# sen-ye/dmvae

Measured on AMD Instinct MI355X. Metric: images/sec DMVAE train step @256x256, higher is better.
Workload: dtype bf16

## Files before the change

dmvae_amd/csrc/conv_pp.hip:

```cpp
#include "common.h"
#include "dmvae_hip.h"
#include <cstdlib>
#include <atomic>
#include <mutex>
#include <type_traits>
#include <unordered_map>


namespace dmvae_conv_pp {

struct Args {
  const bf16* x;
  const bf16* w;
  const float* bias;
  const bf16* res;
  void* y;
  int N, Hi, Wi, Cin, Ho, Wo, Cout;
  int ks, act, M, ctiles, total;
  int so, pd, sd;
  int Ml;
  unsigned wsRow, wsTap, wsChunk;
  float* gnpart;
  unsigned* sched;
  unsigned long long* dbg;
};

__device__ __forceinline__ int hswz(int row) { return (row >> 1) & 2; }

__device__ __forceinline__ void divmod_small(int m, int d, float inv_d, bool, int& q, int& r) {
  q = (int)((float)m * inv_d);
  r = m - q * d;
  if (r < 0) { q--; r += d; }
  if (r >= d) { q++; r -= d; }
}

template <int TM, int TP, int WM, int WP, int NBUF, bool UPS, bool OUT_F32, bool KO, bool GEN = false, bool SUB = false, bool DYN = false, bool STATS = false,
          bool HALO = false>
__global__ __launch_bounds__(512) void conv_pp_kernel(Args a) {
#if __HIP_DEVICE_COMPILE__
  constexpr int BM = TM / WM / 32, BP = TP / WP / 32;
  constexpr int TILE_A = TM * 64, TILE_B = TP * 64, SLOT = TILE_A + TILE_B;
  constexpr int NPA = TM >= 128 ? TM / 128 : 1, NPB = TP / 128;
  static_assert(TM >= 128 || HALO, "the 64-row tile exists in the halo form only");
  constexpr int NP = NPA + NPB;
  constexpr int PF = NBUF - 1;
  static_assert(WM * WP == 8 && BM * BP == 8, "8 waves x 8 accumulators");
  static_assert(!HALO || (!UPS && !GEN && !SUB && KO && NBUF == 4), "HALO: plain 3x3, chunk-outer K order");
  constexpr int NPH = NPB + 1;
  constexpr int HALO_B = (TP + 16) * 64;
  constexpr int GROUP = 2 * TILE_A + HALO_B;
  constexpr int EPI_OFF = HALO ? GROUP : 2 * SLOT;
  constexpr int EPI_BYTES = 8 * 32 * (((BM >= 4 ? BM / 2 : BM) * 32) * 4 + 16);
  constexpr int DUMP_OFF = GROUP + (GROUP > EPI_BYTES ? GROUP : EPI_BYTES);
  constexpr bool DIRECT = HALO && !OUT_F32;
  constexpr int BM16 = BM * 2, BP16 = BP * 2;
  extern __shared__ __attribute__((aligned(16))) char smem[];

  const int tid = threadIdx.x, lane = tid & 63;
  const int wave = __builtin_amdgcn_readfirstlane(tid >> 6);
  const int grp = wave >> 2;
  const int wm = wave / WP, wp = wave % WP;
  static_assert(!SUB || (!UPS && !GEN && KO), "SUB: its own instantiation, chunk-outer K order");
  const int T = SUB ? 4 : a.ks * a.ks;
  const int TW = SUB ? 16 : T;
  const int nchunk = a.Cin >> 5;
  const int nK = T * nchunk;

  const unsigned wbytes = (unsigned)a.Cout * TW * a.Cin * 2u;
  const unsigned xbytes = (unsigned)a.N * a.Hi * a.Wi * a.Cin * 2u;
  const int SR = GEN ? ((UPS || a.ks == 1) ? 0 : (a.sd == 2 ? 1 : a.pd)) : 1;
  const int sds = GEN && a.sd == 2 ? 1 : 0;
  const unsigned shift = GEN ? ((!UPS && a.ks != 1) ? (unsigned)(SR * a.Wi + SR) * a.Cin * 2u : 0u)
                             : ((!UPS && (SUB || a.ks == 3)) ? (unsigned)(a.Wi + 1) * a.Cin * 2u : 0u);
  const __amdgpu_buffer_rsrc_t rA = dmvae_buffer_rsrc(a.w, wbytes);
  const __amdgpu_buffer_rsrc_t rB =
      dmvae_buffer_rsrc(reinterpret_cast<const char*>(a.x) - shift, xbytes + shift);

  const int dvw = SUB ? a.Wi : a.Wo;
  const int hw = SUB ? a.Hi * a.Wi : a.Ho * a.Wo;
  const float inv_hw = 1.0f / (float)hw, inv_wo = 1.0f / (float)dvw;
  const bool small_m = a.M < (1 << 24);
  int m0 = 0, n0 = 0;
  int par = 0;
  unsigned voffA[NPA];
  unsigned ctrB[NPB], maskB[NPB], selB[NPB];
  unsigned rowo[UPS ? NPB : 1][3], colo[UPS ? NPB : 1][3];
  unsigned ctrH[HALO ? NPH : 1], mskH[HALO ? NPH : 1];
  int it_ky = 0;
  int it = 0, it_tap = 0, it_ch = 0;
  unsigned soffB_tap = 0;
  auto setup = [&](unsigned work) {
    int lane_s = lane;
    if constexpr (DIRECT) asm volatile("" : "+v"(lane_s));
    const unsigned wid = xcd_remap(work, a.total);
    if constexpr (SUB) {
      const unsigned q = wid / a.ctiles;
      n0 = (int)(wid - q * a.ctiles) * TM;
      par = __builtin_amdgcn_readfirstlane((int)(q & 3u));
      m0 = (int)(q >> 2) * TP;
    } else {
      m0 = (int)(wid / a.ctiles) * TP;
      n0 = (int)(wid % a.ctiles) * TM;
    }
    it = it_tap = it_ch = 0;
    it_ky = 0;
#pragma unroll
    for (int p = 0; p < NPA; p++) {
      const int row = (wave * NPA + p) * 16 + (lane_s >> 2);
      int co = n0 + row;
      if constexpr (DIRECT) {
        constexpr int CW_ = TM / WM;
        const int wmr = row / CW_, rr = row % CW_;
        co = n0 + wmr * CW_ + BM16 * (rr & 15) + (rr >> 4);
      }
      const int c = (lane_s & 3) ^ swz64(row);
      voffA[p] = (co < a.Cout && row < TM) ? (unsigned)co * a.wsRow + c * 16u : SENT;
    }
    if constexpr (HALO) {
#pragma unroll
      for (int q = 0; q < NPH; q++) {
        const int i = (q < NPB ? (wave * NPB + q) * 16 : TP) + (lane_s >> 2);
        const int own = min(max(i - 1, 0), TP - 1);
        const int m = m0 + own;
        const int c = (lane_s & 3) ^ hswz(i);
        unsigned mask = 0;
        if (m < a.M && i < TP + 2 && (q < NPB || wave == 0)) {
          int n, r, y, x;
          divmod_small(m, hw, inv_hw, small_m, n, r);
          divmod_small(r, dvw, inv_wo, small_m, y, x);
          mask = (y > 0 ? 1u : 0u) | 2u | (y < a.Ho - 1 ? 4u : 0u);
          if ((i == 0 && x == 0) || (i == TP + 1 && x == a.Wo - 1)) mask = 0;
        }
        ctrH[q] = (unsigned)(m0 + i) * a.Cin * 2u + c * 16u;
        mskH[q] = mask;
      }
    } else {
#pragma unroll
    for (int p = 0; p < NPB; p++) {
    const int row = (wave * NPB + p) * 16 + (lane_s >> 2);
    const int m = m0 + row;
    const int c = (lane_s & 3) ^ swz64(row);
    unsigned mask = 0;
    ctrB[p] = 0;
    if (m < a.M) {
      int n, r, y, x;
      divmod_small(m, hw, inv_hw, small_m, n, r);
      divmod_small(r, dvw, inv_wo, small_m, y, x);
      int by = y, bx = x;
      if constexpr (SUB) {
        by = y - 1 + (par >> 1); bx = x - 1 + (par & 1);
        const unsigned rm = (by >= 0 ? 0x3u : 0u) | (by + 1 < a.Hi ? 0xCu : 0u);
        const unsigned cm = (bx >= 0 ? 0x5u : 0u) | (bx + 1 < a.Wi ? 0xAu : 0u);
        mask = rm & cm;
      } else if (UPS || !GEN) {
        if (a.ks == 3) {
          const unsigned rm = (y > 0 ? 0x007u : 0u) | 0x038u | (y < a.Ho - 1 ? 0x1C0u : 0u);
          const unsigned cm = (x > 0 ? 0x049u : 0u) | 0x092u | (x < a.Wo - 1 ? 0x124u : 0u);
          mask = rm & cm;
        } else {
          mask = 1;
        }
      } else if (a.ks == 1) {
        mask = 1;
      } else {
        const int y0 = y * a.so - a.pd, x0 = x * a.so - a.pd;
        by = sds ? (y0 + 1) >> 1 : y0;
        bx = sds ? (x0 + 1) >> 1 : x0;
        unsigned rmk = 0, cmk = 0;
#pragma unroll
        for (int k = 0; k < 4; k++) {
          if (k < a.ks) {
            const bool ry = sds ? (((y0 + k) & 1) == 0 && (unsigned)(by + (k >> 1)) < (unsigned)a.Hi) : (unsigned)(by + k) < (unsigned)a.Hi;
            const bool rx = sds ? (((x0 + k) & 1) == 0 && (unsigned)(bx + (k >> 1)) < (unsigned)a.Wi) : (unsigned)(bx + k) < (unsigned)a.Wi;
            rmk |= (unsigned)ry << k;
            cmk |= (unsigned)rx << k;
          }
        }
#pragma unroll
        for (int k = 0; k < 4; k++)
          if (k < a.ks && ((rmk >> k) & 1u)) mask |= cmk << (k * a.ks);
      }
      if (UPS) {
#pragma unroll
        for (int k = 0; k < 3; k++) {
          const int yy = min(max(y + k - 1, 0), a.Ho - 1) >> 1, xx = min(max(x + k - 1, 0), a.Wo - 1) >> 1;
          rowo[UPS ? p : 0][k] = (unsigned)((n * a.Hi + yy) * a.Wi) * a.Cin * 2u + c * 16u;
          colo[UPS ? p : 0][k] = (unsigned)xx * a.Cin * 2u;
        }
        if (a.ks != 3) ctrB[p] = rowo[UPS ? p : 0][1] + colo[UPS ? p : 0][1];
      } else {
        if constexpr (GEN) ctrB[p] = (unsigned)((n * a.Hi + by + SR) * a.Wi + bx + SR) * a.Cin * 2u + c * 16u;
        else if constexpr (SUB) ctrB[p] = (unsigned)((n * a.Hi + by + 1) * a.Wi + bx + 1) * a.Cin * 2u + c * 16u;
        else ctrB[p] = (unsigned)((n * a.Hi + y) * a.Wi + x) * a.Cin * 2u + c * 16u;
      }
    }
    maskB[p] = mask;
    selB[p] = SENT;
  }
    }
  };

  const int kg = lane >> 5;
  int aoff[BM16], boff[BP16];
#pragma unroll
  for (int i = 0; i < BM16; i++) {
    const int row = wm * (TM / WM) + i * 16 + (lane & 15);
    aoff[i] = row * 64 + (((lane >> 4) ^ swz64(row)) << 4);
  }
#pragma unroll
  for (int j = 0; j < BP16; j++) {
    const int row = wp * (TP / WP) + j * 16 + (lane & 15);
    boff[j] = TILE_A + row * 64 + (((lane >> 4) ^ swz64(row)) << 4);
  }

  f32x4 acc[BM16][BP16];

  auto new_tap = [&]() {
    int ky, kx;
    if constexpr (GEN) {
      ky = a.ks == 3 ? it_tap / 3 : (a.ks == 4 ? it_tap >> 2 : 1); kx = a.ks == 3 ? it_tap - (it_tap / 3) * 3 : (a.ks == 4 ? it_tap & 3 : 1);
      soffB_tap = (!UPS && a.ks != 1) ? (unsigned)((ky >> sds) * a.Wi + (kx >> sds)) * a.Cin * 2u : 0u;
    } else if constexpr (SUB) {
      ky = it_tap >> 1; kx = it_tap & 1;
      soffB_tap = (unsigned)(ky * a.Wi + kx) * a.Cin * 2u;
    } else {
      ky = a.ks == 3 ? it_tap / 3 : 1; kx = a.ks == 3 ? it_tap - (it_tap / 3) * 3 : 1;
      soffB_tap = (!UPS && a.ks == 3) ? (unsigned)(ky * a.Wi + kx) * a.Cin * 2u : 0u;
    }
#pragma unroll
    for (int p = 0; p < NPB; p++) {
      unsigned v = ctrB[p];
      if (UPS && a.ks == 3) {
        const unsigned ro = ky == 0 ? rowo[UPS ? p : 0][0] : (ky == 1 ? rowo[UPS ? p : 0][1] : rowo[UPS ? p : 0][2]);
        const unsigned co = kx == 0 ? colo[UPS ? p : 0][0] : (kx == 1 ? colo[UPS ? p : 0][1] : colo[UPS ? p : 0][2]);
        v = ro + co;
      }
      selB[p] = ((maskB[p] >> it_tap) & 1u) ? v : SENT;
    }
  };
  auto issue = [&](int slot) {
    const bool live = it < nK;
    if (live && (KO || it_ch == 0)) new_tap();
    unsigned soA = (unsigned)it_tap * a.wsTap + (unsigned)it_ch * a.wsChunk;
    if constexpr (SUB)
      soA = (unsigned)((((par >> 1) + (it_tap & 2)) << 2) + (par & 1) + ((it_tap & 1) << 1)) * a.wsTap + (unsigned)it_ch * a.wsChunk;
    unsigned soB = soffB_tap + (unsigned)it_ch * 64u;
    constexpr bool live_b = true;
    if constexpr (GEN) {
      soA = (unsigned)__builtin_amdgcn_readfirstlane((int)soA);
      soB = (unsigned)__builtin_amdgcn_readfirstlane((int)soB);
    }
#pragma unroll
    for (int p = 0; p < NPA; p++)
      __builtin_amdgcn_raw_ptr_buffer_load_lds(rA, LPTR(smem + slot + (wave * NPA + p) * 1024), 16, live ? voffA[p] : SENT, soA, 0, 0);
#pragma unroll
    for (int p = 0; p < NPB; p++)
      __builtin_amdgcn_raw_ptr_buffer_load_lds(rB, LPTR(smem + slot + TILE_A + (wave * NPB + p) * 1024), 16, (live && live_b) ? selB[p] : SENT, soB, 0, 0);
    it++;
    if (KO) {
      if (++it_tap == T) { it_tap = 0; it_ch++; }
    } else {
      if (++it_ch == nchunk) { it_ch = 0; it_tap++; }
    }
  };

  auto issue_h = [&](auto KXc) __attribute__((always_inline)) {
    constexpr int KX = decltype(KXc)::value;
    const bool live = it < nK;
    const unsigned soA = (unsigned)(it_ky * 3 + KX) * a.wsTap + (unsigned)it_ch * a.wsChunk;
    const int isl = it;
    const int da = ((isl >> 1) & 1) * GROUP + (isl & 1) * TILE_A;
#pragma unroll
    for (int p = 0; p < NPA; p++)
      __builtin_amdgcn_raw_ptr_buffer_load_lds(rA, LPTR(smem + ((wave * NPA + p) * 16 < TM ? da + (wave * NPA + p) * 1024 : DUMP_OFF)), 16, live ? voffA[p] : SENT, soA, 0, 0);
    if constexpr (KX == 0) {
      const unsigned soH = (unsigned)(it_ky * a.Wi) * a.Cin * 2u + (unsigned)it_ch * 64u;
      const int dh = ((it_ch + it_ky) & 1) * GROUP + 2 * TILE_A;
#pragma unroll
      for (int q = 0; q < NPH; q++) {
        const unsigned v = (live && ((mskH[HALO ? q : 0] >> it_ky) & 1u)) ? ctrH[HALO ? q : 0] : SENT;
        const int dst = q < NPB ? dh + (wave * NPB + q) * 1024 : (wave == 0 ? dh + TP * 64 : DUMP_OFF);
        __builtin_amdgcn_raw_ptr_buffer_load_lds(rB, LPTR(smem + dst), 16, v, soH, 0, 0);
      }
    }
    it++;
    if constexpr (KX == 2) {
      if (++it_ky == 3) { it_ky = 0; it_ch++; }
    }
  };
  using K0_ = std::integral_constant<int, 0>; using K1_ = std::integral_constant<int, 1>; using K2_ = std::integral_constant<int, 2>;

  auto stamp = [&](unsigned work, int k) {
    if (a.dbg && tid == 0) a.dbg[(size_t)work * 8 + k] = __builtin_amdgcn_s_memtime();
  };
  auto claim = [&]() {
    if (tid == 0) {
      const unsigned x = blockIdx.x & 7u, first = gridDim.x >> 3;
      unsigned flat = 0xFFFFFFFFu;
      for (unsigned k = 0; k < 8u; k++) {
        const unsigned xx = (x + k) & 7u;
        const unsigned cnt = ((unsigned)a.total >> 3) + (xx < ((unsigned)a.total & 7u) ? 1u : 0u);
        const unsigned j = first + atomicAdd(a.sched + xx, 1u);
        if (j < cnt) { flat = j * 8u + xx; break; }
      }
      __hip_atomic_store(a.sched + 16 + blockIdx.x, flat, __ATOMIC_RELEASE, __HIP_MEMORY_SCOPE_WORKGROUP);
    }
  };
  stamp(blockIdx.x, 0);
  setup(blockIdx.x);
  stamp(blockIdx.x, 1);
  if constexpr (HALO) {
    issue_h(K0_{}); issue_h(K1_{}); issue_h(K2_{});
  } else {
#pragma unroll
    for (int u = 0; u < PF; u++) issue(u * SLOT);
  }
  for (unsigned work = blockIdx.x; work < (unsigned)a.total;) {
  const int m0c = m0, n0c = n0;
  const int parc = par;
  if constexpr (DYN) claim();
  int boffk[HALO ? 3 : 1][HALO ? BP16 : 1];
  if constexpr (HALO) {
    int lane_h = lane;
    asm volatile("" : "+v"(lane_h));
#pragma unroll
    for (int j = 0; j < BP16; j++) {
      const int prow = wp * (TP / WP) + j * 16 + (lane_h & 15);
      int q, x;
      divmod_small(m0c + prow, dvw, inv_wo, small_m, q, x);
      const int zoff = (TP + 2) * 64 + ((lane_h >> 4) << 4);
#pragma unroll
      for (int k = 0; k < 3; k++) {
        const int h = prow + k;
        const int off = h * 64 + (((lane_h >> 4) ^ hswz(h)) << 4);
        boffk[HALO ? k : 0][HALO ? j : 0] = (k == 0 && x == 0) || (k == 2 && x == a.Wo - 1) ? zoff : off;
      }
    }
  }
#pragma unroll
  for (int i = 0; i < BM16; i++)
#pragma unroll
    for (int j = 0; j < BP16; j++)
#pragma unroll
      for (int r = 0; r < 4; r++) acc[i][j][r] = 0.f;
  wait_vmcnt<HALO ? 2 * NPA : (PF - 1) * NP>();
  __builtin_amdgcn_s_barrier();
  stamp(work, 2);
  if (grp == 1) __builtin_amdgcn_s_setprio(1);
  if (grp == 1) __builtin_amdgcn_s_barrier();

  bf16x8 af[BM16], bfr[BP16];
  int slot_rd = 0, slot_wr = PF * SLOT;
  unsigned next_dyn = 0;
  if constexpr (HALO) {
    int ka = 0, sh = 2 * TILE_A;
    auto ktile = [&](auto KXc) __attribute__((always_inline)) {
      constexpr int KX = decltype(KXc)::value;
      const char* sa = smem + ((ka >> 1) & 1) * GROUP + (ka & 1) * TILE_A;
      const char* sb = smem + sh;
#pragma unroll
      for (int j = 0; j < BP16; j++) bfr[j] = *reinterpret_cast<const bf16x8*>(sb + boffk[HALO ? KX : 0][HALO ? j : 0]);
#pragma unroll
      for (int i = 0; i < BM16; i++) af[i] = *reinterpret_cast<const bf16x8*>(sa + aoff[i]);
      issue_h(KXc);
      ka++;
      if constexpr (KX == 2) sh = sh == 2 * TILE_A ? GROUP + 2 * TILE_A : 2 * TILE_A;
      wait_vmcnt<KX == 2 ? 2 * NPA : 2 * NPA + NPH>();
      __builtin_amdgcn_s_waitcnt(0xC07F);
      asm volatile("" ::: "memory");
      __builtin_amdgcn_sched_barrier(0);
      __builtin_amdgcn_s_barrier();
      __builtin_amdgcn_sched_barrier(0);
#pragma unroll
      for (int i = 0; i < BM16; i++)
#pragma unroll
        for (int j = 0; j < BP16; j++) {
          if constexpr (DIRECT) asm volatile("v_mfma_f32_16x16x32_bf16 %0, %1, %2, %0" : "+a"(acc[i][j]) : "v"(bfr[j]), "v"(af[i]));
          else asm volatile("v_mfma_f32_16x16x32_bf16 %0, %1, %2, %0" : "+a"(acc[i][j]) : "v"(af[i]), "v"(bfr[j]));
        }
      __builtin_amdgcn_sched_barrier(0);
      __builtin_amdgcn_s_barrier();
      __builtin_amdgcn_sched_barrier(0);
    };
#pragma unroll 1
    for (int t = 0; t < nK; t += 3) { ktile(K0_{}); ktile(K1_{}); ktile(K2_{}); }
  } else {
#pragma unroll 1
  for (int t = 0; t < nK; t++) {
    const char* sb = smem + slot_rd;
#pragma unroll
    for (int j = 0; j < BP16; j++) bfr[j] = *reinterpret_cast<const bf16x8*>(sb + boff[j]);
#pragma unroll
    for (int i = 0; i < BM16; i++) af[i] = *reinterpret_cast<const bf16x8*>(sb + aoff[i]);
    issue(slot_wr);
    slot_rd = slot_rd + SLOT == NBUF * SLOT ? 0 : slot_rd + SLOT;
    slot_wr = slot_wr + SLOT == NBUF * SLOT ? 0 : slot_wr + SLOT;
    wait_vmcnt<(PF - 1) * NP>();
    __builtin_amdgcn_s_waitcnt(0xC07F);
    asm volatile("" ::: "memory");
    __builtin_amdgcn_sched_barrier(0);
    __builtin_amdgcn_s_barrier();
    __builtin_amdgcn_sched_barrier(0);
#pragma unroll
    for (int i = 0; i < BM16; i++)
#pragma unroll
      for (int j = 0; j < BP16; j++)
        asm volatile("v_mfma_f32_16x16x32_bf16 %0, %1, %2, %0" : "+a"(acc[i][j]) : "v"(af[i]), "v"(bfr[j]));
    __builtin_amdgcn_sched_barrier(0);
    __builtin_amdgcn_s_barrier();
    __builtin_amdgcn_sched_barrier(0);
  }
  }
  stamp(work, 3);
  if (grp == 0) __builtin_amdgcn_s_barrier();
  if constexpr (DYN) next_dyn = __hip_atomic_load(a.sched + 16 + blockIdx.x, __ATOMIC_ACQUIRE, __HIP_MEMORY_SCOPE_WORKGROUP);
  wait_vmcnt<0>();
  asm volatile("s_nop 15\n\ts_nop 15" ::: "memory");

  __builtin_amdgcn_s_barrier();
  stamp(work, 6);
  const unsigned next = DYN ? (unsigned)__builtin_amdgcn_readfirstlane((int)next_dyn) : work + gridDim.x;
  const bool has_next = next < (unsigned)a.total;
  if constexpr (DIRECT) {
    typedef unsigned u32x4 __attribute__((ext_vector_type(4)));
    typedef unsigned u32x2 __attribute__((ext_vector_type(2)));
    constexpr int CL = BM16;
    constexpr int NQD = CL / 4;
    static_assert(CL == 8 || CL == 4, "DIRECT: 8 or 4 couts per lane");
    int lane_o = lane;
    asm volatile("" : "+v"(lane_o));
    const int cc = lane_o & 15, gq = lane_o >> 4;
    const int col = n0c + wm * (TM / WM) + CL * cc;
    const bool c_ok = col < a.Cout;
    const __amdgpu_buffer_rsrc_t rY = dmvae_buffer_rsrc(a.y, (unsigned)a.M * (unsigned)a.Cout * 2u);
    const __amdgpu_buffer_rsrc_t rBias = dmvae_buffer_rsrc(a.bias, a.bias ? (unsigned)a.Cout * 4u : 0u);
    float bsv[CL];
    {
      const unsigned vo = c_ok ? (unsigned)col * 4u : SENT;
#pragma unroll
      for (int h = 0; h < NQD; h++) {
        const u32x4 b4 = __builtin_amdgcn_raw_buffer_load_b128(rBias, vo == SENT ? SENT : vo + 16u * h, 0, 0);
        const f32x4 bf = *reinterpret_cast<const f32x4*>(&b4);
#pragma unroll
        for (int e = 0; e < 4; e++) bsv[4 * h + e] = bf[e];
      }
    }
    if (has_next) {
      stamp(next, 0);
      setup(next);
      stamp(next, 1);
    } else {
      it = (nK + 3) & ~3;
      it_ky = it_ch = 0;
    }
    issue_h(K0_{});
    stamp(work, 7);
    float s1[STATS ? NQD : 1], s2[STATS ? NQD : 1];
    if constexpr (STATS) {
#pragma unroll
      for (int h = 0; h < NQD; h++) { s1[h] = 0.f; s2[h] = 0.f; }
    }
    const unsigned vbase = c_ok ? ((unsigned)(m0c + wp * (TP / WP) + 4 * gq) * (unsigned)a.Cout + (unsigned)col) * 2u : SENT;
    const unsigned rstep = (unsigned)a.Cout * 2u;
    auto body = [&](auto RESc, auto ACTc) __attribute__((always_inline)) {
      constexpr bool RES = decltype(RESc)::value;
      constexpr int ACTC = decltype(ACTc)::value;
      const __amdgpu_buffer_rsrc_t rR = dmvae_buffer_rsrc(a.res, RES ? (unsigned)a.M * (unsigned)a.Cout * 2u : 0u);
      typedef std::conditional_t<CL == 8, u32x4, u32x2> rvec;
      rvec rnx[RES ? 4 : 1];
      auto fetch = [&](int j, int r) {
        if constexpr (RES) {
          if constexpr (CL == 8) rnx[RES ? r : 0] = __builtin_amdgcn_raw_buffer_load_b128(rR, vbase, (unsigned)(j * 16 + r) * rstep, 2);
          else rnx[RES ? r : 0] = __builtin_amdgcn_raw_buffer_load_b64(rR, vbase, (unsigned)(j * 16 + r) * rstep, 2);
        }
      };
#pragma unroll
      for (int r = 0; r < 4; r++) fetch(0, r);
#pragma unroll
      for (int j = 0; j < BP16; j++) {
#pragma unroll
        for (int r = 0; r < 4; r++) {
          float v[CL];
#pragma unroll
          for (int i = 0; i < CL; i++) {
            float x;
            asm volatile("v_accvgpr_read_b32 %0, %1" : "=v"(x) : "a"(acc[i][j][r]));
            v[i] = x + bsv[i];
          }
          const int act = ACTC >= 0 ? ACTC : a.act;
          if constexpr (RES) {
            float rf[CL];
            {
              const rvec rv = rnx[RES ? r : 0];
#pragma unroll
              for (int h = 0; h < CL / 2; h++) {
                const unsigned wd = rv[h];
                const bf16x2 b2 = *reinterpret_cast<const bf16x2*>(&wd);
                rf[2 * h] = (float)b2[0]; rf[2 * h + 1] = (float)b2[1];
              }
            }
            if (j + 1 < BP16) fetch(j + 1, r);
            if (act == 3) {
#pragma unroll
              for (int e = 0; e < CL; e++) v[e] = rf[e] > 0.f ? v[e] : 0.f;
            } else {
#pragma unroll
              for (int e = 0; e < CL; e++) v[e] += rf[e];
            }
          }
          if (act == 1) {
#pragma unroll
            for (int e = 0; e < CL; e++) v[e] = v[e] * sigmoidf_(v[e]);
          } else if (act == 2) {
#pragma unroll
            for (int e = 0; e < CL; e++) v[e] = v[e] > 0.f ? v[e] : 0.f;
          } else if (act == 4) {
#pragma unroll
            for (int e = 0; e < CL; e++) v[e] = v[e] > 0.f ? v[e] : 0.2f * v[e];
          }
          const unsigned so = (unsigned)(j * 16 + r) * rstep;
          unsigned pk[CL / 2];
#pragma unroll
          for (int h = 0; h < CL / 2; h++) pk[h] = dmvae_pack_bf16x2(v[2 * h], v[2 * h + 1]);
          if constexpr (STATS) {
            const bf16x2 one2 = {(bf16)1.0f, (bf16)1.0f};
#pragma unroll
            for (int h = 0; h < CL / 2; h++) {
              const bf16x2 p2 = *reinterpret_cast<const bf16x2*>(&pk[h]);
              s1[STATS ? h >> 1 : 0] = __builtin_amdgcn_fdot2_f32_bf16(p2, one2, s1[STATS ? h >> 1 : 0], false);
              s2[STATS ? h >> 1 : 0] = __builtin_amdgcn_fdot2_f32_bf16(p2, p2, s2[STATS ? h >> 1 : 0], false);
            }
          }
          if constexpr (CL == 8) {
            const u32x4 o = {pk[0], pk[1], pk[2], pk[3]};
            __builtin_amdgcn_raw_buffer_store_b128(o, rY, vbase, so, 2 );
            asm volatile("s_nop 0" :: "v"(o));
          } else {
            const u32x2 o = {pk[0], pk[1]};
            __builtin_amdgcn_raw_buffer_store_b64(o, rY, vbase, so, 2 );
            asm volatile("s_nop 0" :: "v"(o));
          }
        }
      }
    };
    using T_ = std::true_type; using F_ = std::false_type;
    if (a.res) {
      if (a.act == 0) body(T_{}, std::integral_constant<int, 0>{});
      else if (a.act == 3) body(T_{}, std::integral_constant<int, 3>{});
      else body(T_{}, std::integral_constant<int, -1>{});
    } else {
      if (a.act == 0) body(F_{}, std::integral_constant<int, 0>{});
      else if (a.act == 2) body(F_{}, std::integral_constant<int, 2>{});
      else body(F_{}, std::integral_constant<int, -1>{});
    }
    if constexpr (STATS) {
      const size_t trow = (size_t)(m0c / TP) * WP + wp;
#pragma unroll
      for (int h = 0; h < NQD; h++) {
        float t1 = s1[STATS ? h : 0], t2 = s2[STATS ? h : 0];
        t1 += __shfl_xor(t1, 16, 64); t2 += __shfl_xor(t2, 16, 64);
        t1 += __shfl_xor(t1, 32, 64); t2 += __shfl_xor(t2, 32, 64);
        const int cq = col + 4 * h;
        if (gq == 0 && cq < a.Cout) *reinterpret_cast<f32x2*>(a.gnpart + (trow * (a.Cout >> 2) + (cq >> 2)) * 2) = f32x2{t1, t2};
      }
    }
  } else {
    constexpr int EH = BM >= 4 ? BM / 2 : BM;
    constexpr int NH = BM / EH;
    constexpr int CWH = EH * 32;
    constexpr int ROWB = CWH * 4 + 16;
    constexpr int LPR = CWH / 8, RPI = 64 / LPR;
    constexpr int NI = 32 / RPI;
    constexpr unsigned ES = OUT_F32 ? 4u : 2u;
    static_assert(!STATS || !OUT_F32, "STATS: statistics of the bf16 result");
    typedef unsigned u32x4 __attribute__((ext_vector_type(4)));
    char* reg = smem + EPI_OFF + wave * (32 * ROWB);
    int lane_o = lane;
    asm volatile("" : "+v"(lane_o));
    const int cl = lane_o % LPR, rg = lane_o / LPR;
    const unsigned mout = SUB ? 4u * (unsigned)a.M : (unsigned)a.M;
    const __amdgpu_buffer_rsrc_t rY = dmvae_buffer_rsrc(a.y, mout * (unsigned)a.Cout * ES);
    const __amdgpu_buffer_rsrc_t rBias = dmvae_buffer_rsrc(a.bias, a.bias ? (unsigned)a.Cout * 4u : 0u);
    f32x4 bias_lo[NH], bias_hi[NH];
#pragma unroll
    for (int hh = 0; hh < NH; hh++) {
      const int cb = n0c + wm * (TM / WM) + hh * CWH + cl * 8;
      const unsigned vo = cb < a.Cout ? (unsigned)cb * 4u : SENT;
      const u32x4 b0 = __builtin_amdgcn_raw_buffer_load_b128(rBias, vo, 0, 0), b1 = __builtin_amdgcn_raw_buffer_load_b128(rBias, vo + 16u, 0, 0);
      bias_lo[hh] = *reinterpret_cast<const f32x4*>(&b0);
      bias_hi[hh] = *reinterpret_cast<const f32x4*>(&b1);
    }
    if (has_next) {
      stamp(next, 0);
      setup(next);
      stamp(next, 1);
    } else {
      it = HALO ? (nK + 3) & ~3 : nK;
      it_ky = it_ch = 0;
    }
    if constexpr (HALO) issue_h(K0_{}); else issue(0);
    stamp(work, 7);
    float sacc[STATS ? NH : 1][2][2];
    if constexpr (STATS) {
#pragma unroll
      for (int i = 0; i < NH * 4; i++) (&sacc[0][0][0])[i] = 0.f;
    }
    auto body = [&](auto RESc, auto ACTc) __attribute__((always_inline)) {
      constexpr bool RES = decltype(RESc)::value;
      constexpr int ACTC = decltype(ACTc)::value;
      const __amdgpu_buffer_rsrc_t rR = dmvae_buffer_rsrc(a.res, RES ? mout * (unsigned)a.Cout * 2u : 0u);
#pragma unroll
      for (int hh = 0; hh < NH; hh++) {
        if (n0c + wm * (TM / WM) + hh * CWH >= a.Cout) continue;
        const int cb = n0c + wm * (TM / WM) + hh * CWH + cl * 8;
        const bool c_ok = cb < a.Cout;
        const unsigned row_e = (unsigned)(m0c + wp * (TP / WP) + rg) * (unsigned)a.Cout + (unsigned)cb;
        const unsigned ybase = c_ok ? row_e * ES : SENT, rbase = c_ok ? row_e * 2u : SENT;
        const unsigned ystep = (unsigned)(RPI * a.Cout) * ES, rstep = (unsigned)(RPI * a.Cout) * 2u;
        auto sub_off = [&](int j, int it2) -> unsigned {
          const int m = m0c + wp * (TP / WP) + j * 32 + it2 * RPI + rg;
          int n, r, y, x;
          divmod_small(m, hw, inv_hw, small_m, n, r);
          divmod_small(r, dvw, inv_wo, small_m, y, x);
          const unsigned mo = (unsigned)((n * a.Ho + 2 * y + (parc >> 1)) * a.Wo + 2 * x + (parc & 1));
          return (m < a.M && c_ok) ? mo * (unsigned)a.Cout + (unsigned)cb : SENT;
        };
        auto stage = [&](int j) {
#pragma unroll
          for (int i = 0; i < EH * 2; i++)
#pragma unroll
            for (int jb = 0; jb < 2; jb++)
              *reinterpret_cast<f32x4*>(reg + (jb * 16 + (lane_o & 15)) * ROWB + (i * 16 + 4 * (lane_o >> 4)) * 4) = acc[hh * EH * 2 + i][j * 2 + jb];
        };
        constexpr int NPART = RES ? 2 : 1, NQ = NI / NPART;
        u32x4 r8s[RES ? 2 : 1][RES ? NI : 1];
        auto fetch = [&](int j, int h2) {
          if constexpr (RES) {
#pragma unroll
            for (int it2 = h2 * NQ; it2 < (h2 + 1) * NQ; it2++) {
              if constexpr (SUB) {
                const unsigned eo = sub_off(j, it2);
                r8s[j & 1][it2] = __builtin_amdgcn_raw_buffer_load_b128(rR, eo == SENT ? SENT : eo * 2u, 0, 2);
              } else {
                r8s[j & 1][it2] = __builtin_amdgcn_raw_buffer_load_b128(rR, rbase, (unsigned)(j * NI + it2) * rstep, 2);
              }
            }
          }
        };
#pragma unroll
        for (int h2 = 0; h2 < NPART; h2++) fetch(0, h2);
        stage(0);
#pragma unroll
        for (int j = 0; j < BP; j++) {
#pragma unroll
          for (int h2 = 0; h2 < NPART; h2++) {
          f32x4 lo[NQ], hi[NQ];
#pragma unroll
          for (int q = 0; q < NQ; q++) {
            const int px = (h2 * NQ + q) * RPI + rg;
            lo[q] = *reinterpret_cast<const f32x4*>(reg + px * ROWB + cl * 32);
            hi[q] = *reinterpret_cast<const f32x4*>(reg + px * ROWB + cl * 32 + 16);
          }
          if (j + 1 < BP) {
            if (h2 == NPART - 1) stage(j + 1);
            fetch(j + 1, h2);
          }
          u32x4 keep[OUT_F32 ? 2 * NQ : NQ];
#pragma unroll
          for (int q = 0; q < NQ; q++) {
            const int it2 = h2 * NQ + q;
            f32x4 v0 = lo[q] + bias_lo[hh], v1 = hi[q] + bias_hi[hh];
            float v[8] = {v0[0], v0[1], v0[2], v0[3], v1[0], v1[1], v1[2], v1[3]};
            const int act = ACTC >= 0 ? ACTC : a.act;
            if constexpr (RES) {
              const bf16x8 r8 = *reinterpret_cast<const bf16x8*>(&r8s[j & 1][it2]);
              if (act == 3) {
#pragma unroll
                for (int e = 0; e < 8; e++) v[e] = (float)r8[e] > 0.f ? v[e] : 0.f;
              } else {
#pragma unroll
                for (int e = 0; e < 8; e++) v[e] += (float)r8[e];
              }
            }
            if (act == 1) {
#pragma unroll
              for (int e = 0; e < 8; e++) v[e] = v[e] * sigmoidf_(v[e]);
            } else if (act == 2) {
#pragma unroll
              for (int e = 0; e < 8; e++) v[e] = v[e] > 0.f ? v[e] : 0.f;
            } else if (act == 4) {
#pragma unroll
              for (int e = 0; e < 8; e++) v[e] = v[e] > 0.f ? v[e] : 0.2f * v[e];
            }
            unsigned voff = ybase, soff = (unsigned)(j * NI + it2) * ystep;
            if constexpr (SUB) {
              const unsigned eo = sub_off(j, it2);
              voff = eo == SENT ? SENT : eo * ES;
              soff = 0u;
            }
            if constexpr (OUT_F32) {
              const f32x4 o0 = {v[0], v[1], v[2], v[3]}, o1 = {v[4], v[5], v[6], v[7]};
              keep[2 * q] = *reinterpret_cast<const u32x4*>(&o0);
              keep[2 * q + 1] = *reinterpret_cast<const u32x4*>(&o1);
              __builtin_amdgcn_raw_buffer_store_b128(keep[2 * q], rY, voff, soff, 0);
              __builtin_amdgcn_raw_buffer_store_b128(keep[2 * q + 1], rY, voff + 16u, soff, 0);
            } else {
              const u32x4 o = {dmvae_pack_bf16x2(v[0], v[1]), dmvae_pack_bf16x2(v[2], v[3]), dmvae_pack_bf16x2(v[4], v[5]), dmvae_pack_bf16x2(v[6], v[7])};
              if constexpr (STATS) {
                const bf16x2 one2 = {(bf16)1.0f, (bf16)1.0f};
#pragma unroll
                for (int pr = 0; pr < 4; pr++) {
                  const unsigned pw = o[pr];
                  const bf16x2 p2 = *reinterpret_cast<const bf16x2*>(&pw);
                  float& s1 = sacc[STATS ? hh : 0][pr >> 1][0];
                  float& s2 = sacc[STATS ? hh : 0][pr >> 1][1];
                  s1 = __builtin_amdgcn_fdot2_f32_bf16(p2, one2, s1, false);
                  s2 = __builtin_amdgcn_fdot2_f32_bf16(p2, p2, s2, false);
                }
              }
              keep[q] = o;
              __builtin_amdgcn_raw_buffer_store_b128(o, rY, voff, soff, 2);
            }
          }
#pragma unroll
          for (int q = 0; q < (OUT_F32 ? 2 * NQ : NQ); q++) asm volatile("s_nop 0" :: "v"(keep[q]));
          }
        }
      }
    };
    using T_ = std::true_type; using F_ = std::false_type;
    if (a.res) {
      if (a.act == 0) body(T_{}, std::integral_constant<int, 0>{});
      else if (a.act == 3) body(T_{}, std::integral_constant<int, 3>{});
      else body(T_{}, std::integral_constant<int, -1>{});
    } else {
      if (a.act == 0) body(F_{}, std::integral_constant<int, 0>{});
      else if (a.act == 2) body(F_{}, std::integral_constant<int, 2>{});
      else body(F_{}, std::integral_constant<int, -1>{});
    }
    if constexpr (STATS) {
      const size_t trow = (size_t)(SUB ? (m0c / TP) * 4 + parc : m0c / TP) * WP + wp;
#pragma unroll
      for (int hh = 0; hh < NH; hh++)
#pragma unroll
        for (int qd = 0; qd < 2; qd++) {
          float s1 = sacc[STATS ? hh : 0][qd][0], s2 = sacc[STATS ? hh : 0][qd][1];
#pragma unroll
          for (int off = LPR; off < 64; off <<= 1) { s1 += __shfl_xor(s1, off, 64); s2 += __shfl_xor(s2, off, 64); }
          const int cq = n0c + wm * (TM / WM) + hh * CWH + lane_o * 8 + qd * 4;
          if (lane_o < LPR && cq < a.Cout) *reinterpret_cast<f32x2*>(a.gnpart + (trow * (a.Cout >> 2) + (cq >> 2)) * 2) = f32x2{s1, s2};
        }
    }
  }
  if (has_next) { if constexpr (HALO) issue_h(K1_{}); else issue(SLOT); }
  stamp(work, 4);
  wait_vmcnt<HALO ? NPA : NP>();
  stamp(work, 5);
  __builtin_amdgcn_s_barrier();
  if (has_next) { if constexpr (HALO) issue_h(K2_{}); else issue(2 * SLOT); }
  work = next;
  }
  if constexpr (DYN) {
    if (tid == 0 && atomicAdd(a.sched + 8, 1u) == gridDim.x - 1) {
#pragma unroll
      for (int k = 0; k < 9; k++) __hip_atomic_store(a.sched + k, 0u, __ATOMIC_RELAXED, __HIP_MEMORY_SCOPE_AGENT);
    }
  }
#endif
}

constexpr int SCHED_WORDS = 16 + 512, SCHED_SLOTS = 32;
__device__ unsigned g_sched[SCHED_SLOTS * SCHED_WORDS];

static unsigned* sched_for(hipStream_t st) {
  static std::mutex mu;
  static std::unordered_map<unsigned long long, int> slot;
  static std::unordered_map<int, unsigned*> base;
  static std::unordered_map<int, int> used;
  int dev = 0;
  if (hipGetDevice(&dev) != hipSuccess) { (void)hipGetLastError(); return nullptr; }
  std::lock_guard<std::mutex> lk(mu);
  auto b = base.find(dev);
  if (b == base.end()) {
    unsigned* p = nullptr;
    if (hipGetSymbolAddress(reinterpret_cast<void**>(&p), HIP_SYMBOL(g_sched)) != hipSuccess) { (void)hipGetLastError(); return nullptr; }
    b = base.emplace(dev, p).first;
  }
  const unsigned long long key = ((unsigned long long)(unsigned)dev << 56) ^ (unsigned long long)reinterpret_cast<uintptr_t>(st);
  auto it = slot.find(key);
  if (it == slot.end()) {
    int& n = used[dev];
    if (n >= SCHED_SLOTS) return nullptr;
    it = slot.emplace(key, n++).first;
  }
  return b->second + (size_t)it->second * SCHED_WORDS;
}

static std::atomic<int> g_dynamic{-1};
static bool dynamic_on() {
  const int v = g_dynamic.load(std::memory_order_relaxed);
  if (v >= 0) return v != 0;
  static const bool env = [] { const char* e = getenv("DMVAE_PP_DYNAMIC"); return e ? atoi(e) != 0 : false; }();
  return env;
}

template <int TM, int TP, int WM, int WP, int NBUF, bool UPS, bool F32, bool KO, bool GEN = false, bool SUB = false, bool DYN = false, bool STATS = false,
          bool HALO = false>
int launch(Args a, hipStream_t st) {
  a.ctiles = (a.Cout + TM - 1) / TM;
  a.total = ((a.M + TP - 1) / TP) * a.ctiles * (SUB ? 4 : 1);
  constexpr int persist = 256;
  const unsigned grid = (persist > 0 && a.total > persist) ? (unsigned)persist : (unsigned)a.total;
  if constexpr (!DYN && !UPS && KO && !F32) {
    if (dynamic_on() && grid == 256u && (unsigned)a.total > grid) {
      a.sched = sched_for(st);
      if (a.sched) return launch<TM, TP, WM, WP, NBUF, UPS, F32, KO, GEN, SUB, true, STATS, HALO>(a, st);
    }
  }
  constexpr int cwh = (TM / WM / 32 >= 4) ? TM / WM / 2 : TM / WM;
  constexpr int ring = NBUF * (TM + TP) * 64, epi = 2 * (TM + TP) * 64 + 8 * 32 * (cwh * 4 + 16);
  constexpr int group = 2 * TM * 64 + (TP + 16) * 64, epi_h = 8 * 32 * (cwh * 4 + 16);
  constexpr int lds = HALO ? group + (group > epi_h ? group : epi_h) + 1024 : (ring > epi ? ring : epi);
  DMVAE_LDS_OPTIN(lds, conv_pp_kernel<TM, TP, WM, WP, NBUF, UPS, F32, KO, GEN, SUB, DYN, STATS, HALO>);
  hipLaunchKernelGGL((conv_pp_kernel<TM, TP, WM, WP, NBUF, UPS, F32, KO, GEN, SUB, DYN, STATS, HALO>), dim3(grid), dim3(512), lds, st, a);
  DMVAE_CHECK_LAUNCH();
  return 0;
}

static constexpr int halo_mode() { return 3; }
static constexpr bool korder_on() { return true; }
static bool halo_for(int ks, int cout, bool plain, bool ups, bool f32) {
  const int h = halo_mode();
  return plain && !ups && !f32 && ks == 3 && h != 0 && korder_on() && (cout > 128 || (h & 2));
}

template <bool UPS, bool F32>
int pick(const Args& a, hipStream_t st, bool gen) {
  if constexpr (!UPS) {
    if (gen) {
      if (a.Cout <= 128) return launch<128, 512, 2, 4, 4, false, F32, true, true>(a, st);
      return launch<256, 256, 2, 4, 4, false, F32, true, true>(a, st);
    }
  }
  if constexpr (UPS) {
    if (a.Cout <= 128) return launch<128, 512, 2, 4, 4, UPS, F32, false>(a, st);
    return launch<256, 256, 2, 4, 4, UPS, F32, false>(a, st);
  } else {
    if constexpr (!F32) {
      if (halo_for(a.ks, a.Cout, !gen, UPS, F32)) {
        if (a.Cout > 128) return a.gnpart ? launch<256, 256, 2, 4, 4, false, false, true, false, false, false, true, true>(a, st)
                                          : launch<256, 256, 2, 4, 4, false, false, true, false, false, false, false, true>(a, st);
        if (a.Cout <= 64 && !a.gnpart)
          return launch<64, 1024, 1, 8, 4, false, false, true, false, false, false, false, true>(a, st);
        return a.gnpart ? launch<128, 512, 2, 4, 4, false, false, true, false, false, false, true, true>(a, st)
                        : launch<128, 512, 2, 4, 4, false, false, true, false, false, false, false, true>(a, st);
      }
      if (a.gnpart) {
        if (a.Cout <= 128) return launch<128, 512, 2, 4, 4, false, false, true, false, false, false, true>(a, st);
        return launch<256, 256, 2, 4, 4, false, false, true, false, false, false, true>(a, st);
      }
    }
    if (a.Cout <= 128) return launch<128, 512, 2, 4, 4, UPS, F32, true>(a, st);
    return launch<256, 256, 2, 4, 4, UPS, F32, true>(a, st);
  }
}

}

static unsigned long long* g_dbg = nullptr;
extern "C" void dmvae_debug_timing(void* buf) { g_dbg = (unsigned long long*)buf; }

__global__ __launch_bounds__(64) void occupy_kernel(unsigned long long ticks) {
  extern __shared__ char occ[];
  occ[threadIdx.x] = 0;
  const unsigned long long t0 = wall_clock64();
  while (wall_clock64() - t0 < ticks) __builtin_amdgcn_s_sleep(32);
}
extern "C" int dmvae_set_dynamic(int on) {
  dmvae_conv_pp::g_dynamic.store(on < 0 ? -1 : (on != 0), std::memory_order_relaxed);
  return dmvae_conv_pp::dynamic_on() ? 1 : 0;
}

extern "C" int dmvae_debug_occupy(int blocks, int lds_bytes, int microseconds, hipStream_t stream) {
  DMVAE_LDS_OPTIN(160 * 1024, occupy_kernel);
  hipLaunchKernelGGL(occupy_kernel, dim3(blocks), dim3(64), lds_bytes, stream, (unsigned long long)microseconds * 100ull);
  DMVAE_CHECK_LAUNCH();
  return 0;
}

int dmvae_conv_geometry(const dmvae_conv_desc* d, int* ho, int* wo, int* so, int* pd, int* sd, int* fl);

extern "C" int dmvae_conv_halo_applies(const dmvae_conv_desc* d) {
  using namespace dmvae_conv_pp;
  if (!d) return 0;
  int ho, wo, so, pd, sd, fl;
  if (dmvae_conv_geometry(d, &ho, &wo, &so, &pd, &sd, &fl) != 0) return 0;
  const bool plain = !(d->upsample == 2 || d->stride == 2 || d->ks == 4 || d->transposed);
  const long long M = (long long)d->n * ho * wo;
  const long long xbytes = (long long)d->n * d->h * d->w * d->cin * 2;
  const long long wbytes = (long long)d->cout * d->ks * d->ks * d->cin * 2;
  constexpr long long min_m = 16384;
  if (d->cin % 32 != 0 || d->cout < 64 || d->cout % 8 != 0 || M < min_m || xbytes + (1ll << 22) >= (1ll << 31) || wbytes >= (1ll << 31)) return 0;
  if (M >= (1ll << 24) || M * d->cout * (d->out_f32 ? 4 : 2) >= (1ll << 31)) return 0;
  return halo_for(d->ks, d->cout, plain, fl != 0, d->out_f32 != 0) ? 1 : 0;
}

extern "C" int dmvae_conv_kmajor_applies(const dmvae_conv_desc* d) {
  using namespace dmvae_conv_pp;
  if (!d) return 0;
  int ho, wo, so, pd, sd, fl;
  if (dmvae_conv_geometry(d, &ho, &wo, &so, &pd, &sd, &fl) != 0) return 0;
  const bool plain = !(d->upsample == 2 || d->stride == 2 || d->ks == 4 || d->transposed);
  const long long M = (long long)d->n * ho * wo;
  const long long xbytes = (long long)d->n * d->h * d->w * d->cin * 2;
  const long long wbytes = (long long)d->cout * d->ks * d->ks * d->cin * 2;
  constexpr long long min_m = 16384;
  if (d->cin % 32 != 0 || d->cout < 64 || d->cout % 8 != 0 || M < min_m || xbytes + (1ll << 22) >= (1ll << 31) || wbytes >= (1ll << 31)) return 0;
  if (M >= (1ll << 24) || M * d->cout * (d->out_f32 ? 4 : 2) >= (1ll << 31)) return 0;
  return 1;
}

int dmvae_conv_pp_try(const void* x, const void* w, const void* bias, const void* residual, void* y, const dmvae_conv_desc* d,
                      hipStream_t stream, float* gnpart, int gn_groups, int* gn_tp) {
  if (gn_tp) *gn_tp = 0;
  using namespace dmvae_conv_pp;
  int ho, wo, so, pd, sd, fl;
  if (dmvae_conv_geometry(d, &ho, &wo, &so, &pd, &sd, &fl) != 0) return 1;
  const bool plain = !(d->upsample == 2 || d->stride == 2 || d->ks == 4 || d->transposed);
  const bool sub = d->transposed && d->ks == 4 && d->stride == 2;
  const int ups = fl ? 1 : 0;
  const long long M = (long long)d->n * ho * wo;
  const long long xbytes = (long long)d->n * d->h * d->w * d->cin * 2;
  const long long wbytes = (long long)d->cout * d->ks * d->ks * d->cin * 2;
  constexpr long long min_m = 16384;
  if (d->cin % 32 != 0 || d->cout < 64 || d->cout % 8 != 0 || M < min_m || xbytes + (1ll << 22) >= (1ll << 31) || wbytes >= (1ll << 31)) return 1;
  if (M >= (1ll << 24)) return 1;
  if (M * d->cout * (d->out_f32 ? 4 : 2) >= (1ll << 31)) return 1;
  if (d->w_layout != 0 && d->w_layout != 1) {
    dmvae_set_error("conv2d_nhwc_fwd: w_layout %d (0 = tap-major, 1 = K-tile-major where dmvae_conv_kmajor_applies(d) is 1)", d->w_layout);
    return -1;
  }
  Args a;
  a.wsRow = d->w_layout ? 64u : (unsigned)(d->ks * d->ks * d->cin) * 2u;
  a.wsTap = d->w_layout ? (unsigned)d->cout * 64u : (unsigned)d->cin * 2u;
  a.wsChunk = d->w_layout ? (unsigned)(d->ks * d->ks) * (unsigned)d->cout * 64u : 64u;
  a.x = (const bf16*)x; a.w = (const bf16*)w; a.bias = (const float*)bias; a.res = (const bf16*)residual; a.y = y;
  a.N = d->n; a.Hi = d->h; a.Wi = d->w; a.Cin = d->cin; a.Cout = d->cout;
  a.Ho = ho; a.Wo = wo; a.so = so; a.pd = pd; a.sd = sd;
  a.ks = d->ks; a.act = d->act; a.M = (int)M; a.ctiles = 0; a.dbg = g_dbg;
  a.Ml = d->n * d->h * d->w;
  a.gnpart = nullptr;
  if (gnpart && gn_tp && !d->out_f32 && (plain || sub) && !ups && gn_groups > 0 && d->cout % gn_groups == 0 && (d->cout / gn_groups) % 4 == 0) {
    const int tp = d->cout <= 128 ? 512 : 256;
    const long long per_image = sub ? (long long)d->h * d->w : (long long)ho * wo;
    if (per_image % tp == 0) { a.gnpart = gnpart; *gn_tp = tp; }
  }
  a.sched = nullptr;
  const bool f32 = d->out_f32 != 0;
  if (sub) {
    a.M = a.Ml;
    if (a.gnpart) {
      if (a.Cout <= 128) return launch<128, 512, 2, 4, 4, false, false, true, false, true, false, true>(a, stream);
      return launch<256, 256, 2, 4, 4, false, false, true, false, true, false, true>(a, stream);
    }
    if (a.Cout <= 128) return f32 ? launch<128, 512, 2, 4, 4, false, true, true, false, true>(a, stream) : launch<128, 512, 2, 4, 4, false, false, true, false, true>(a, stream);
    return f32 ? launch<256, 256, 2, 4, 4, false, true, true, false, true>(a, stream) : launch<256, 256, 2, 4, 4, false, false, true, false, true>(a, stream);
  }
  if (ups) return f32 ? pick<true, true>(a, stream, false) : pick<true, false>(a, stream, false);
  return f32 ? pick<false, true>(a, stream, !plain) : pick<false, false>(a, stream, !plain);
}
```

Baseline: 501.3.

## Reuse halo B fragments in registers across the three horizontal conv taps

When the output width allows it, the halo conv path remaps pixel rows so each lane owns BP16 consecutive output pixels. It then loads BP16+2 B fragments from LDS once per kernel row and reuses them, shifted, for all three horizontal taps, where before it reloaded BP16 fragments per tap. The halo prefetch is reordered so weight loads are issued after the halo loads, and the epilogue row strides are changed to match the new pixel mapping. This cuts LDS read traffic in the MFMA loop, at the cost of more live VGPRs and new index arithmetic that has to stay correct at image edges.

```diff
diff --git a/dmvae_amd/csrc/conv_pp.hip b/dmvae_amd/csrc/conv_pp.hip
--- a/dmvae_amd/csrc/conv_pp.hip
+++ b/dmvae_amd/csrc/conv_pp.hip
@@ -23,6 +23,7 @@
   float* gnpart;
   unsigned* sched;
   unsigned long long* dbg;
+  int reuse;
 };
 
 __device__ __forceinline__ int hswz(int row) { return (row >> 1) & 2; }
@@ -119,10 +120,16 @@
     if constexpr (HALO) {
 #pragma unroll
       for (int q = 0; q < NPH; q++) {
-        const int i = (q < NPB ? (wave * NPB + q) * 16 : TP) + (lane_s >> 2);
+        const int L = (q < NPB ? (wave * NPB + q) * 16 : TP) + (lane_s >> 2);
+        int i = L;
+        if (a.reuse) {
+          constexpr int RG = TP / BP16;
+          if (q < NPB) i = (L % RG) * BP16 + L / RG;
+          else i = L == TP ? TP : (L == TP + 8 ? TP + 1 : TP + 2);
+        }
         const int own = min(max(i - 1, 0), TP - 1);
         const int m = m0 + own;
-        const int c = (lane_s & 3) ^ hswz(i);
+        const int c = (lane_s & 3) ^ hswz(L);
         unsigned mask = 0;
         if (m < a.M && i < TP + 2 && (q < NPB || wave == 0)) {
           int n, r, y, x;
@@ -264,16 +271,20 @@
     }
   };
 
-  auto issue_h = [&](auto KXc) __attribute__((always_inline)) {
+  auto issue_h = [&](auto KXc, auto LATEc) __attribute__((always_inline)) {
     constexpr int KX = decltype(KXc)::value;
+    constexpr bool LATE = decltype(LATEc)::value;
     const bool live = it < nK;
     const unsigned soA = (unsigned)(it_ky * 3 + KX) * a.wsTap + (unsigned)it_ch * a.wsChunk;
     const int isl = it;
     const int da = ((isl >> 1) & 1) * GROUP + (isl & 1) * TILE_A;
-#pragma unroll
-    for (int p = 0; p < NPA; p++)
-      __builtin_amdgcn_raw_ptr_buffer_load_lds(rA, LPTR(smem + ((wave * NPA + p) * 16 < TM ? da + (wave * NPA + p) * 1024 : DUMP_OFF)), 16, live ? voffA[p] : SENT, soA, 0, 0);
-    if constexpr (KX == 0) {
+    auto a_pieces = [&]() __attribute__((always_inline)) {
+#pragma unroll
+      for (int p = 0; p < NPA; p++)
+        __builtin_amdgcn_raw_ptr_buffer_load_lds(rA, LPTR(smem + ((wave * NPA + p) * 16 < TM ? da + (wave * NPA + p) * 1024 : DUMP_OFF)), 16, live ? voffA[p] : SENT, soA, 0, 0);
+    };
+    if constexpr (!LATE) a_pieces();
+    if constexpr (KX == (LATE ? 1 : 0)) {
       const unsigned soH = (unsigned)(it_ky * a.Wi) * a.Cin * 2u + (unsigned)it_ch * 64u;
       const int dh = ((it_ch + it_ky) & 1) * GROUP + 2 * TILE_A;
 #pragma unroll
@@ -283,6 +294,7 @@
         __builtin_amdgcn_raw_ptr_buffer_load_lds(rB, LPTR(smem + dst), 16, v, soH, 0, 0);
       }
     }
+    if constexpr (LATE) a_pieces();
     it++;
     if constexpr (KX == 2) {
       if (++it_ky == 3) { it_ky = 0; it_ch++; }
@@ -310,7 +322,7 @@
   setup(blockIdx.x);
   stamp(blockIdx.x, 1);
   if constexpr (HALO) {
-    issue_h(K0_{}); issue_h(K1_{}); issue_h(K2_{});
+    issue_h(K0_{}, std::false_type{}); issue_h(K1_{}, std::false_type{}); issue_h(K2_{}, std::false_type{});
   } else {
 #pragma unroll
     for (int u = 0; u < PF; u++) issue(u * SLOT);
@@ -323,6 +335,20 @@
   if constexpr (HALO) {
     int lane_h = lane;
     asm volatile("" : "+v"(lane_h));
+    if (a.reuse) {
+      constexpr int RG = TP / BP16;
+      const int p = lane_h & 15, r0 = wp * 16 + p;
+      int q, x;
+      divmod_small(m0c + wp * (TP / WP) + BP16 * p, dvw, inv_wo, small_m, q, x);
+      const int zoff = (TP + 2) * 64 + ((lane_h >> 4) << 4);
+      auto ro = [&](int L) { return L * 64 + (((lane_h >> 4) ^ hswz(L)) << 4); };
+#pragma unroll
+      for (int b = 0; b < BP16 + 2; b++) {
+        const int L = b < BP16 ? b * RG + r0 : (r0 + 1 < RG ? (b - BP16) * RG + r0 + 1 : TP + 8 * (b - BP16));
+        const bool edge = (b == 0 && x == 0) || (b == BP16 + 1 && x + BP16 == a.Wo);
+        boffk[HALO ? b / BP16 : 0][HALO ? b % BP16 : 0] = edge ? zoff : ro(L);
+      }
+    } else
 #pragma unroll
     for (int j = 0; j < BP16; j++) {
       const int prow = wp * (TP / WP) + j * 16 + (lane_h & 15);
@@ -354,18 +380,27 @@
   unsigned next_dyn = 0;
   if constexpr (HALO) {
     int ka = 0, sh = 2 * TILE_A;
-    auto ktile = [&](auto KXc) __attribute__((always_inline)) {
+    bf16x8 hb[BP16 + 2];
+    auto ktile = [&](auto KXc, auto REc) __attribute__((always_inline)) {
       constexpr int KX = decltype(KXc)::value;
+      constexpr bool RE = decltype(REc)::value;
       const char* sa = smem + ((ka >> 1) & 1) * GROUP + (ka & 1) * TILE_A;
       const char* sb = smem + sh;
-#pragma unroll
-      for (int j = 0; j < BP16; j++) bfr[j] = *reinterpret_cast<const bf16x8*>(sb + boffk[HALO ? KX : 0][HALO ? j : 0]);
+      if constexpr (RE) {
+        if constexpr (KX == 0) {
+#pragma unroll
+          for (int b = 0; b < BP16 + 2; b++) hb[b] = *reinterpret_cast<const bf16x8*>(sb + boffk[HALO ? b / BP16 : 0][HALO ? b % BP16 : 0]);
+        }
+      } else {
+#pragma unroll
+        for (int j = 0; j < BP16; j++) hb[j] = *reinterpret_cast<const bf16x8*>(sb + boffk[HALO ? KX : 0][HALO ? j : 0]);
+      }
 #pragma unroll
       for (int i = 0; i < BM16; i++) af[i] = *reinterpret_cast<const bf16x8*>(sa + aoff[i]);
-      issue_h(KXc);
+      issue_h(KXc, REc);
       ka++;
       if constexpr (KX == 2) sh = sh == 2 * TILE_A ? GROUP + 2 * TILE_A : 2 * TILE_A;
-      wait_vmcnt<KX == 2 ? 2 * NPA : 2 * NPA + NPH>();
+      wait_vmcnt<(RE ? KX != 1 : KX == 2) ? 2 * NPA : 2 * NPA + NPH>();
       __builtin_amdgcn_s_waitcnt(0xC07F);
       asm volatile("" ::: "memory");
       __builtin_amdgcn_sched_barrier(0);
@@ -375,15 +410,20 @@
       for (int i = 0; i < BM16; i++)
 #pragma unroll
         for (int j = 0; j < BP16; j++) {
-          if constexpr (DIRECT) asm volatile("v_mfma_f32_16x16x32_bf16 %0, %1, %2, %0" : "+a"(acc[i][j]) : "v"(bfr[j]), "v"(af[i]));
-          else asm volatile("v_mfma_f32_16x16x32_bf16 %0, %1, %2, %0" : "+a"(acc[i][j]) : "v"(af[i]), "v"(bfr[j]));
+          if constexpr (DIRECT) asm volatile("v_mfma_f32_16x16x32_bf16 %0, %1, %2, %0" : "+a"(acc[i][j]) : "v"(hb[RE ? j + KX : j]), "v"(af[i]));
+          else asm volatile("v_mfma_f32_16x16x32_bf16 %0, %1, %2, %0" : "+a"(acc[i][j]) : "v"(af[i]), "v"(hb[RE ? j + KX : j]));
         }
       __builtin_amdgcn_sched_barrier(0);
       __builtin_amdgcn_s_barrier();
       __builtin_amdgcn_sched_barrier(0);
     };
+    if (DIRECT && a.reuse) {
 #pragma unroll 1
-    for (int t = 0; t < nK; t += 3) { ktile(K0_{}); ktile(K1_{}); ktile(K2_{}); }
+      for (int t = 0; t < nK; t += 3) { ktile(K0_{}, std::true_type{}); ktile(K1_{}, std::true_type{}); ktile(K2_{}, std::true_type{}); }
+    } else {
+#pragma unroll 1
+      for (int t = 0; t < nK; t += 3) { ktile(K0_{}, std::false_type{}); ktile(K1_{}, std::false_type{}); ktile(K2_{}, std::false_type{}); }
+    }
   } else {
 #pragma unroll 1
   for (int t = 0; t < nK; t++) {
@@ -453,15 +493,16 @@
       it = (nK + 3) & ~3;
       it_ky = it_ch = 0;
     }
-    issue_h(K0_{});
+    issue_h(K0_{}, std::false_type{});
     stamp(work, 7);
     float s1[STATS ? NQD : 1], s2[STATS ? NQD : 1];
     if constexpr (STATS) {
 #pragma unroll
       for (int h = 0; h < NQD; h++) { s1[h] = 0.f; s2[h] = 0.f; }
     }
-    const unsigned vbase = c_ok ? ((unsigned)(m0c + wp * (TP / WP) + 4 * gq) * (unsigned)a.Cout + (unsigned)col) * 2u : SENT;
+    const unsigned vbase = c_ok ? ((unsigned)(m0c + wp * (TP / WP) + (a.reuse ? 4 * BP16 : 4) * gq) * (unsigned)a.Cout + (unsigned)col) * 2u : SENT;
     const unsigned rstep = (unsigned)a.Cout * 2u;
+    const unsigned jstep = a.reuse ? rstep : 16u * rstep, qstep = a.reuse ? (unsigned)BP16 * rstep : rstep;
     auto body = [&](auto RESc, auto ACTc) __attribute__((always_inline)) {
       constexpr bool RES = decltype(RESc)::value;
       constexpr int ACTC = decltype(ACTc)::value;
@@ -470,8 +511,8 @@
       rvec rnx[RES ? 4 : 1];
       auto fetch = [&](int j, int r) {
         if constexpr (RES) {
-          if constexpr (CL == 8) rnx[RES ? r : 0] = __builtin_amdgcn_raw_buffer_load_b128(rR, vbase, (unsigned)(j * 16 + r) * rstep, 2);
-          else rnx[RES ? r : 0] = __builtin_amdgcn_raw_buffer_load_b64(rR, vbase, (unsigned)(j * 16 + r) * rstep, 2);
+          if constexpr (CL == 8) rnx[RES ? r : 0] = __builtin_amdgcn_raw_buffer_load_b128(rR, vbase, (unsigned)j * jstep + (unsigned)r * qstep, 2);
+          else rnx[RES ? r : 0] = __builtin_amdgcn_raw_buffer_load_b64(rR, vbase, (unsigned)j * jstep + (unsigned)r * qstep, 2);
         }
       };
 #pragma unroll
@@ -518,7 +559,7 @@
 #pragma unroll
             for (int e = 0; e < CL; e++) v[e] = v[e] > 0.f ? v[e] : 0.2f * v[e];
           }
-          const unsigned so = (unsigned)(j * 16 + r) * rstep;
+          const unsigned so = (unsigned)j * jstep + (unsigned)r * qstep;
           unsigned pk[CL / 2];
 #pragma unroll
           for (int h = 0; h < CL / 2; h++) pk[h] = dmvae_pack_bf16x2(v[2 * h], v[2 * h + 1]);
@@ -598,7 +639,7 @@
       it = HALO ? (nK + 3) & ~3 : nK;
       it_ky = it_ch = 0;
     }
-    if constexpr (HALO) issue_h(K0_{}); else issue(0);
+    if constexpr (HALO) issue_h(K0_{}, std::false_type{}); else issue(0);
     stamp(work, 7);
     float sacc[STATS ? NH : 1][2][2];
     if constexpr (STATS) {
@@ -752,12 +793,12 @@
         }
     }
   }
-  if (has_next) { if constexpr (HALO) issue_h(K1_{}); else issue(SLOT); }
+  if (has_next) { if constexpr (HALO) issue_h(K1_{}, std::false_type{}); else issue(SLOT); }
   stamp(work, 4);
   wait_vmcnt<HALO ? NPA : NP>();
   stamp(work, 5);
   __builtin_amdgcn_s_barrier();
-  if (has_next) { if constexpr (HALO) issue_h(K2_{}); else issue(2 * SLOT); }
+  if (has_next) { if constexpr (HALO) issue_h(K2_{}, std::false_type{}); else issue(2 * SLOT); }
   work = next;
   }
   if constexpr (DYN) {
@@ -804,9 +845,13 @@
   return env;
 }
 
+static std::atomic<int> g_halo_reuse{-1};
+static int halo_reuse_mode() { return g_halo_reuse.load(std::memory_order_relaxed); }
+
 template <int TM, int TP, int WM, int WP, int NBUF, bool UPS, bool F32, bool KO, bool GEN = false, bool SUB = false, bool DYN = false, bool STATS = false,
           bool HALO = false>
 int launch(Args a, hipStream_t st) {
+  a.reuse = (HALO && !F32 && halo_reuse_mode() != 0 && a.Wo % (TP / WP / 16) == 0) ? 1 : 0;
   a.ctiles = (a.Cout + TM - 1) / TM;
   a.total = ((a.M + TP - 1) / TP) * a.ctiles * (SUB ? 4 : 1);
   constexpr int persist = 256;
@@ -880,6 +925,8 @@
   dmvae_conv_pp::g_dynamic.store(on < 0 ? -1 : (on != 0), std::memory_order_relaxed);
   return dmvae_conv_pp::dynamic_on() ? 1 : 0;
 }
+
+extern "C" void dmvae_debug_conv_halo_reuse(int mode) { dmvae_conv_pp::g_halo_reuse.store(mode < 0 ? -1 : (mode != 0), std::memory_order_relaxed); }
 
 extern "C" int dmvae_debug_occupy(int blocks, int lds_bytes, int microseconds, hipStream_t stream) {
   DMVAE_LDS_OPTIN(160 * 1024, occupy_kernel);
```

After: 504.8, median of 6. About the same (+0.7%).
